# CederGroupHub/sparse-lm

Measured on NVIDIA B200. Metric: cv_grid_fits_per_sec, higher is better.
Workload: dtype f64

## Files before the change

include/sparselm_b200.h:

```cpp
#ifndef SPARSELM_B200_H
#define SPARSELM_B200_H

#include <stddef.h>
#include <stdint.h>

#ifdef __cplusplus
extern "C" {
#endif

#define SLM_MAX_FOLDS 16

typedef struct slm_ctx slm_ctx;

int slm_version(void);
int slm_create(int device, slm_ctx** out);
void slm_destroy(slm_ctx* ctx);
int slm_set_option(slm_ctx* ctx, const char* name, int value);
const char* slm_last_error(const slm_ctx* ctx);
int slm_sm_count(const slm_ctx* ctx);
int64_t slm_launch_count(const slm_ctx* ctx);
int64_t slm_tma_launch_count(const slm_ctx* ctx);
int slm_timing_enable(slm_ctx* ctx, int on);
int slm_timing_read(slm_ctx* ctx, int which, double* total_ms, int64_t* launches, double* flops);
int slm_timing_reset(slm_ctx* ctx);
// ... 104 lines not shown
                      const int32_t* K, const double* const* intercept_dev, int32_t rows_scaled,
                      double* const* yhat_dev, const int64_t* ldy, double* const* out_dev, void* stream);

int slm_cv_score_rows(slm_ctx* ctx, const double* Xa_dev, int64_t lda, int64_t p, int32_t n,
                      const int32_t* const* rows_dev, const int64_t* n_rows, const double* const* B_dev,
                      const int64_t* ldb, const int32_t* K, const double* const* intercept_dev, int32_t rows_scaled,
                      double* const* yhat_dev, const int64_t* ldy, double* const* out_dev, void* stream);

int slm_intercepts(slm_ctx* ctx, const double* G_dev, int64_t pa, int64_t p,
                   const double* B_dev, int64_t ldz, int32_t K, double* intercept_dev,
                   void* stream);

size_t slm_newton_workspace(int64_t p, int32_t n_groups, int32_t k, int n_folds);
int slm_newton_step(slm_ctx* ctx, const double* G_dev, int64_t g_stride, int64_t pa, int64_t p, int n_folds,
                    int32_t k, const int32_t* fold_host, const double* nobs_dev, double* X_dev,
                    const double* W2_dev, const double* D2_dev, const int32_t* gptr_dev, const int32_t* gid_dev,
                    int32_t n_groups, void* work_dev, size_t work_bytes, double* out_dev, void* stream);

int slm_newton_step_l1(slm_ctx* ctx, const double* G_dev, int64_t g_stride, int64_t pa, int64_t p, int n_folds,
                       int32_t k, const int32_t* fold_host, const double* nobs_dev, double* X_dev,
                       const double* W2_dev, const double* D2_dev, const double* W1_dev, const int32_t* gptr_dev,
                       const int32_t* gid_dev, int32_t n_groups, void* work_dev, size_t work_bytes, double* out_dev,
                       void* stream);

size_t slm_gram_cg_workspace(int64_t p);
int slm_gram_cg(slm_ctx* ctx, const double* G_dev, int64_t pa, int64_t p, const double* shift_dev,
                double tol, int32_t max_iter, void* work_dev, size_t work_bytes, double* X8_dev,
                int32_t* iters_host, double* relres_host, void* stream);

int slm_gram_apply(slm_ctx* ctx, const double* G_dev, int64_t g_stride, int64_t pa, int64_t p,
                   int n_folds, const int32_t* K, const double* Z_dev, int64_t ldz,
                   double* GZ_dev, void* stream);

size_t slm_rowsparse_workspace(int64_t p, int64_t ldz, int n_folds);
int slm_gram_apply_rowsparse(slm_ctx* ctx, const double* G_dev, int64_t g_stride, int64_t pa,
                             int64_t p, int n_folds, const int32_t* K, const double* Z_dev,
                             int64_t ldz, double* GZ_dev, int chunk_w, void* work_dev,
                             size_t work_bytes, void* stream);

int slm_apply_stats(slm_ctx* ctx, double* executed_flops, double* dense_flops);

int slm_group_whiten_factors(slm_ctx* ctx, const double* G_dev, int64_t pa, int64_t p,
                             const int32_t* gptr_dev, const int64_t* wptr_dev, int32_t n_groups,
                             const double* shift_dev, double* W_dev, double* scratch_dev,
                             int32_t* info_dev, void* stream);
int slm_gram_whiten(slm_ctx* ctx, const double* G_dev, int64_t pa, int64_t p,
                    const int32_t* gptr_dev, const int64_t* wptr_dev, int32_t n_groups,
                    const double* W_dev, const double* ridge_dev, double ridge_scale,
                    double* tmp_dev, double* Gout_dev, void* stream);
int slm_coef_unwhiten(slm_ctx* ctx, const double* Bg_dev, int64_t p, int64_t ldz, int32_t K,
                      const int32_t* gptr_dev, const int64_t* wptr_dev, int32_t n_groups,
                      const double* W_dev, double* B_dev, void* stream);

#ifdef __cplusplus
}
#endif
#endif
```

sparselm_b200/_build.py:

```python

from __future__ import annotations

import os
import shutil
import subprocess

_PKG = os.path.dirname(os.path.abspath(__file__))
CSRC = os.path.join(_PKG, "csrc")
LIB_DIR = os.path.join(_PKG, "lib")
LIB_PATH = os.path.join(LIB_DIR, "libsparselm_b200.so")
SOURCES = ["engine.cu"]
HEADERS = ["gemm_f64.cuh", "gemm_f64_tma.cuh", "solver_kernels.cuh", "whiten_kernels.cuh", "cg_kernels.cuh", "coop_kernels.cuh", "newton_kernels.cuh", os.path.join("..", "..", "include", "sparselm_b200.h")]

NVCC_FLAGS = [
    "-gencode", "arch=compute_100a,code=sm_100a",
    "-O3", "-lineinfo", "-std=c++17",
    "-Xcompiler", "-fPIC", "-shared",
]


def find_nvcc() -> str:
    nvcc = shutil.which("nvcc") or "/usr/local/cuda/bin/nvcc"
    if not os.path.exists(nvcc):
        raise RuntimeError("nvcc not found: the sparselm_b200 CUDA engine cannot be built")
    return nvcc


def is_stale() -> bool:
    if not os.path.exists(LIB_PATH):
        return True
    t = os.path.getmtime(LIB_PATH)
    deps = [os.path.join(CSRC, s) for s in SOURCES] + [os.path.join(CSRC, h) for h in HEADERS]
    return any(os.path.getmtime(d) > t for d in deps)


def build(force: bool = False, verbose: bool = False) -> str:
    if not force and not is_stale():
        return LIB_PATH
    os.makedirs(LIB_DIR, exist_ok=True)
    cmd = [find_nvcc(), *NVCC_FLAGS, "-o", LIB_PATH] + [os.path.join(CSRC, s) for s in SOURCES]
    if verbose:
        cmd.insert(1, "-Xptxas")
        cmd.insert(2, "-v")
    res = subprocess.run(cmd, capture_output=True, text=True)
    if res.returncode != 0:
# ... 9 lines not shown
```

sparselm_b200/_lib.py:

```python

from __future__ import annotations

import ctypes
import os

from . import _build

SLM_MAX_FOLDS = 16

c_i32, c_i64, c_dbl, c_vp, c_sz = (
    ctypes.c_int32, ctypes.c_int64, ctypes.c_double, ctypes.c_void_p, ctypes.c_size_t,
)


class SlmBatch(ctypes.Structure):

    _fields_ = [
        ("n_folds", c_i32),
        ("n_groups", c_i32),
        ("p", c_i64),
        ("pa", c_i64),
        ("ldz", c_i64),
        ("G_dev", c_vp),
        ("g_stride", c_i64),
# ... 35 lines not shown
    "slm_tma_launch_count": (c_i64, [c_vp]),
    "slm_timing_enable": (ctypes.c_int, [c_vp, ctypes.c_int]),
    "slm_timing_read": (ctypes.c_int, [c_vp, ctypes.c_int, ctypes.POINTER(c_dbl), ctypes.POINTER(c_i64), ctypes.POINTER(c_dbl)]),
    "slm_timing_reset": (ctypes.c_int, [c_vp]),
    "slm_padded_cols": (c_i64, [c_i64]),
    "slm_pack_design": (ctypes.c_int, [c_vp, c_vp, c_i64, c_vp, c_vp, c_vp, c_vp, c_i64, c_i64, c_vp, c_i64, c_vp]),
    "slm_gram_blocks": (ctypes.c_int, [c_vp, c_vp, c_i64, ctypes.POINTER(c_i64), ctypes.c_int, c_vp, c_vp]),
    "slm_gram_block_add": (ctypes.c_int, [c_vp, c_vp, c_i64, c_i64, c_i64, c_vp, c_vp]),
    "slm_gram_rows_update": (ctypes.c_int, [c_vp, c_vp, c_i64, c_i64, ctypes.c_int, ctypes.POINTER(c_i64), c_vp, c_vp, c_i64,
                                            ctypes.c_int, ctypes.c_int, c_vp]),
    "slm_gram_complement": (ctypes.c_int, [c_vp, c_vp, ctypes.c_int, c_i64, c_vp, c_vp]),
    "slm_tri_size": (c_i64, [c_i64]),
    "slm_tri_pack": (ctypes.c_int, [c_vp, c_vp, c_i64, c_i64, ctypes.c_int, c_vp, c_vp]),
    "slm_tri_unpack": (ctypes.c_int, [c_vp, c_vp, c_i64, ctypes.c_int, c_vp, c_i64, c_vp]),
    "slm_tri_complement": (ctypes.c_int, [c_vp, c_vp, c_i64, ctypes.c_int, c_vp, c_i64, c_vp]),
    "slm_gram_allreduce": (ctypes.c_int, [c_vp, c_vp, c_vp, c_i64, c_i64, ctypes.c_int, c_vp, c_vp]),
    "slm_allreduce_sum": (ctypes.c_int, [c_vp, c_vp, c_vp, c_i64, c_vp]),
    "slm_gather_results": (ctypes.c_int, [c_vp, c_vp, c_vp, c_vp, c_i64, c_vp]),
    "slm_tma_probe": (ctypes.c_int, [c_vp, c_vp, c_i64, c_i64, c_i32, c_i32, ctypes.POINTER(c_i32), c_vp, c_vp]),
    "slm_gram_center": (ctypes.c_int, [c_vp, c_vp, c_i64, c_i64, c_vp]),
    "slm_gram_gather": (ctypes.c_int, [c_vp, c_vp, c_i64, c_i64, c_vp, c_i64, c_vp, c_i64, c_vp]),
    "slm_lipschitz_workspace": (c_sz, [c_i64, ctypes.c_int]),
    "slm_lipschitz": (ctypes.c_int, [c_vp, c_vp, c_i64, c_i64, c_i64, ctypes.c_int, ctypes.c_int, c_vp, ctypes.POINTER(c_dbl), c_vp]),
    "slm_lipschitz_dev": (ctypes.c_int, [c_vp, c_vp, c_i64, c_i64, c_i64, ctypes.c_int, ctypes.c_int, c_vp, c_vp, c_vp]),
    "slm_solve_workspace": (c_sz, [c_i64, c_i64, ctypes.c_int, ctypes.c_int]),
    "slm_solve_batch": (ctypes.c_int, [c_vp, ctypes.POINTER(SlmBatch), c_vp]),
    "slm_adaptive_update": (ctypes.c_int, [c_vp, c_vp, c_i64, c_i64, c_i32, c_i32, c_vp, c_vp, c_vp, c_vp, c_vp, c_dbl, c_vp, c_vp, c_vp, c_vp]),
    "slm_fold_back": (ctypes.c_int, [c_vp, c_vp, c_vp, c_vp, c_i64, c_i64, c_i32, c_vp, c_vp]),
    "slm_cv_score": (ctypes.c_int, [c_vp, c_vp, c_i64, c_i64, c_i64, c_i64, c_vp, c_i64, c_i32, c_vp, c_i32, c_vp, c_vp, c_vp]),
    "slm_cv_score_many": (ctypes.c_int, [c_vp, c_vp, c_i64, c_i64, c_i32, c_vp, c_vp, c_vp, c_vp, c_vp, c_vp, c_i32, c_vp, c_vp, c_vp, c_vp]),
    "slm_cv_score_rows": (ctypes.c_int, [c_vp, c_vp, c_i64, c_i64, c_i32, c_vp, c_vp, c_vp, c_vp, c_vp, c_vp, c_i32, c_vp, c_vp, c_vp, c_vp]),
    "slm_intercepts": (ctypes.c_int, [c_vp, c_vp, c_i64, c_i64, c_vp, c_i64, c_i32, c_vp, c_vp]),
    "slm_gram_apply": (ctypes.c_int, [c_vp, c_vp, c_i64, c_i64, c_i64, ctypes.c_int, ctypes.POINTER(c_i32), c_vp, c_i64, c_vp, c_vp]),
    "slm_newton_workspace": (c_sz, [c_i64, c_i32, c_i32, ctypes.c_int]),
    "slm_newton_step": (ctypes.c_int, [c_vp, c_vp, c_i64, c_i64, c_i64, ctypes.c_int, c_i32, ctypes.POINTER(c_i32), c_vp, c_vp,
                                       c_vp, c_vp, c_vp, c_vp, c_i32, c_vp, c_sz, c_vp, c_vp]),
    "slm_newton_step_l1": (ctypes.c_int, [c_vp, c_vp, c_i64, c_i64, c_i64, ctypes.c_int, c_i32, ctypes.POINTER(c_i32), c_vp,
                                          c_vp, c_vp, c_vp, c_vp, c_vp, c_vp, c_i32, c_vp, c_sz, c_vp, c_vp]),
    "slm_gram_cg_workspace": (c_sz, [c_i64]),
    "slm_gram_cg": (ctypes.c_int, [c_vp, c_vp, c_i64, c_i64, c_vp, c_dbl, c_i32, c_vp, c_sz, c_vp, ctypes.POINTER(c_i32), ctypes.POINTER(c_dbl), c_vp]),
    "slm_rowsparse_workspace": (c_sz, [c_i64, c_i64, ctypes.c_int]),
    "slm_gram_apply_rowsparse": (ctypes.c_int, [c_vp, c_vp, c_i64, c_i64, c_i64, ctypes.c_int, ctypes.POINTER(c_i32), c_vp, c_i64, c_vp, ctypes.c_int, c_vp, c_sz, c_vp]),
    "slm_apply_stats": (ctypes.c_int, [c_vp, ctypes.POINTER(c_dbl), ctypes.POINTER(c_dbl)]),
    "slm_group_whiten_factors": (ctypes.c_int, [c_vp, c_vp, c_i64, c_i64, c_vp, c_vp, c_i32, c_vp, c_vp, c_vp, c_vp, c_vp]),
    "slm_gram_whiten": (ctypes.c_int, [c_vp, c_vp, c_i64, c_i64, c_vp, c_vp, c_i32, c_vp, c_vp, c_dbl, c_vp, c_vp, c_vp]),
    "slm_coef_unwhiten": (ctypes.c_int, [c_vp, c_vp, c_i64, c_i64, c_i32, c_vp, c_vp, c_i32, c_vp, c_vp, c_vp]),
}

_lib = None


def lib_path() -> str:
    return os.environ.get("SLM_B200_LIB") or _build.LIB_PATH


def load():
    global _lib
    if _lib is not None:
        return _lib
    path = lib_path()
    if not os.path.exists(path):
        raise RuntimeError(
            f"sparselm_b200 CUDA engine not built ({path} missing): run "
            "`python -c 'import __graft_entry__ as g; g.build()'` -- there is no CPU fallback"
        )
    lib = ctypes.CDLL(path)
# ... 7 lines not shown
```

sparselm_b200/csrc/engine.cu:

```cuda
#include <cuda_runtime.h>
#include <math.h>
#include <stdint.h>
#include <stdio.h>
#include <stdlib.h>
#include <string.h>

#include <algorithm>
#include <string>
#include <vector>

#include "../../include/sparselm_b200.h"
#include "gemm_f64.cuh"
#include "gemm_f64_tma.cuh"
#include "solver_kernels.cuh"
#include "whiten_kernels.cuh"
#include "cg_kernels.cuh"
#include "coop_kernels.cuh"
#include "newton_kernels.cuh"

using namespace slm;

enum { FAM_GRAM = 0, FAM_APPLY = 1, FAM_PROX = 2, FAM_GAP = 3, FAM_SCORE = 4, FAM_LIPS = 5, FAM_COUNT = 6 };

struct Family {
    std::vector<cudaEvent_t> ev;
    std::vector<cudaEvent_t> pool;
    double ms = 0.0;
    double flops = 0.0;
    int64_t n = 0;
};

constexpr int kMaxScount = 4096;
constexpr int kMaxDevices = 64;

struct slm_ctx {
    int device = 0;
    int sm_count = 148;
    std::string err;
    int64_t launches = 0;
    int64_t tma_launches = 0;
    bool timing = false;
    bool newton_smem_set = false;
    Family fam[FAM_COUNT];
    int* d_counter = nullptr;
    int* h_counter = nullptr;
    int* d_flags = nullptr;
    int n_flags_cap = 0;
    unsigned long long* d_stat = nullptr;
    unsigned long long* h_stat = nullptr;
    unsigned long long* d_ratio = nullptr;
    unsigned long long* h_ratio = nullptr;
    int* h_scount = nullptr;
    double* h_scal = nullptr;
    double apply_exec_flops = 0.0;
    double apply_dense_flops = 0.0;
    int chunk_w = 32;
    bool dense_apply = false;
    bool small_fused = true;
    bool coop = true;
    bool trace = false;
    int coop_max_smem = 0;
    int max_cluster = 16;
    int force_sparse_shape = -1;
    int force_apply_shape = -1;
    int force_syrk_shape = -1;
    bool fused_prox = true;
    bool prox2 = false;
    int tma_mask = 7 + 8;
    void* encode = nullptr;
};

static int fail(slm_ctx* ctx, int code, const std::string& msg) {
    if (ctx) ctx->err = msg;
    return code;
}
#define CUDA_OK(call)                                                                      \
    do {                                                                                   \
        cudaError_t e__ = (call);                                                          \
        if (e__ != cudaSuccess)                                                            \
            return fail(ctx, 100 + (int)e__,                                               \
                        std::string(#call) + ": " + cudaGetErrorString(e__));              \
    } while (0)
#define LAUNCH_OK(name)                                                                    \
    do {                                                                                   \
        cudaError_t e__ = cudaGetLastError();                                              \
        if (e__ != cudaSuccess)                                                            \
            return fail(ctx, 100 + (int)e__, std::string(name) + ": " + cudaGetErrorString(e__)); \
        ctx->launches++;                                                                   \
    } while (0)

struct FamTimer {
    slm_ctx* ctx;
    int fam;
    cudaStream_t s;
    cudaEvent_t e0 = nullptr, e1 = nullptr;
    FamTimer(slm_ctx* c, int f, cudaStream_t st, double flops) : ctx(c), fam(f), s(st) {
        Family& F = ctx->fam[fam];
        F.flops += flops;
        F.n += 1;
// ... 328 lines not shown
        memset(&b, 0, sizeof(b));
        ProblemDims pd[kMaxGemmProblems];
        double flops = 0.0;
        b.n_problems = nf;
        if (g_stride % pa == 0) {
            b.baseP = G;
            b.rowsP = (int64_t)(F - 1) * (g_stride / pa) + pa;
            b.baseQ = Z;
            b.rowsQ = (int64_t)F * p;
        }
        for (int i = 0; i < nf; ++i) {
            int f = f0 + i;
            GemmProblem& pr = b.pr[i];
            pr.P = G + (int64_t)f * g_stride;
            pr.Q = Z + (int64_t)f * p * ldz;
            pr.C = GZ + (int64_t)f * p * ldz;
            pr.ldp = pa;
            pr.ldq = ldz;
            pr.ldc = ldz;
            pr.M = (int)p;
            pr.N = (int)std::min<int64_t>(round_up(K[f], 8), ldz);
            pr.Kd = (int)p;
            pd[i] = {pr.M, pr.N};
            flops += 2.0 * (double)p * (double)p * (double)K[f];
        }
        int sid = pick_shape(kApplyShapes, kNumApplyShapes, pd, nf, ctx->sm_count);
        if (ctx->force_apply_shape >= 0 && ctx->force_apply_shape < kNumApplyShapes) sid = ctx->force_apply_shape;
        FamTimer tm(ctx, family, s, algo_flops >= 0 ? algo_flops : flops);
        cudaError_t e = launch_apply_shape(ctx, sid, b, s);
        if (e != cudaSuccess) return fail(ctx, 100 + (int)e, std::string("gram apply: ") + cudaGetErrorString(e));
        ctx->launches++;
    }
    return 0;
}

static int apply_rowsparse(slm_ctx* ctx, const SolveDev& sp, const int32_t* K, const double* Z, double* GZ,
                           int chunk_w, int ncc, int* sidx, int* scount, cudaStream_t s, double algo_flops) {
    const int F = sp.F;
    const int64_t p = sp.p, ldz = sp.ldz;
    support_list_kernel<<<dim3((unsigned)ncc, (unsigned)F), 1024, 0, s>>>(sp, chunk_w / SC, ncc, sidx, scount,
                                                                          ctx->d_stat);
    LAUNCH_OK("support_list_kernel");
    GemmBatch b;
    ProblemDims pd[kMaxGemmProblems];
    int np = 0;
    double dense = 0.0;
    bool first = true;
    auto flush = [&]() -> int {
        if (np == 0) return 0;
        b.n_problems = np;
        if (sp.g_stride % sp.pa == 0) {
            b.baseP = sp.G;
            b.rowsP = (int64_t)(F - 1) * (sp.g_stride / sp.pa) + sp.pa;
            b.baseQ = Z;
            b.rowsQ = (int64_t)F * p;
        }
        int sid = pick_shape(kSparseShapes, kNumSparseShapes, pd, np, ctx->sm_count);
        if (ctx->force_sparse_shape >= 0 && ctx->force_sparse_shape < 14) sid = ctx->force_sparse_shape;
        FamTimer tm(ctx, FAM_APPLY, s, first ? std::max(algo_flops, 0.0) : 0.0);
        first = false;
        cudaError_t e = launch_sparse_shape(ctx, sid, b, s);
        if (e != cudaSuccess) return fail(ctx, 100 + (int)e, std::string("row-sparse apply: ") + cudaGetErrorString(e));
        ctx->launches++;
        np = 0;
        return 0;
    };
// ... 151 lines not shown
        if (gl < s) red[gl][c] += red[gl + s][c];
        __syncthreads();
    }
    T r = red[0][c];
    __syncthreads();
    return r;
}

__global__ void init_cols_kernel(double* theta, double* tmom, int* flag, int* colmap, int* status, int* n_iter,
                                 const int* skip, long long n, int ldz) {
    long long i = (long long)blockIdx.x * blockDim.x + threadIdx.x;
    if (i >= n) return;
    theta[i] = theta[n + i] = 0.0;
    tmom[i] = tmom[n + i] = 1.0;
    colmap[i] = (int)(i % ldz);
    if (skip && skip[i]) {
        flag[i] = 3;
        return;
    }
    flag[i] = 0;
    if (status) status[i] = -1;
    if (n_iter) n_iter[i] = 0;
}

constexpr int PN_LANES = 128;
__global__ void __launch_bounds__(8 * PN_LANES) power_norm_kernel(double* __restrict__ V, const double* __restrict__ W,
                                                                  int p, double* __restrict__ lam, int init) {
    const int f = blockIdx.x;
    const int c = threadIdx.x & 7, r = threadIdx.x >> 3;
    double* Vf = V + (long long)f * p * 8;
    const double* Wf = W + (long long)f * p * 8;
    __shared__ double red[3][PN_LANES][8];
    if (init) {
        for (int j = r; j < p; j += PN_LANES) {
            unsigned h = (unsigned)(j * 8 + c) * 2654435761u + 12345u * (unsigned)(f + 1);
            h ^= h >> 15;
            h *= 2246822519u;
            h ^= h >> 13;
            Vf[(long long)j * 8 + c] = ((double)(h & 0xffffff) / 8388608.0) - 1.0;
        }
        if (threadIdx.x == 0) lam[f] = 0.0;
        return;
    }
    double vw = 0.0, ww = 0.0, vv = 0.0;
    for (int j = r; j < p; j += PN_LANES) {
        double v = Vf[(long long)j * 8 + c], w = Wf[(long long)j * 8 + c];
        vw += v * w;
        ww += w * w;
        vv += v * v;
    }
    red[0][r][c] = vw;
    red[1][r][c] = ww;
    red[2][r][c] = vv;
    __syncthreads();
    for (int s = PN_LANES / 2; s > 0; s >>= 1) {
        if (r < s) {
            red[0][r][c] += red[0][r + s][c];
            red[1][r][c] += red[1][r + s][c];
            red[2][r][c] += red[2][r + s][c];
        }
        __syncthreads();
    }
    vw = red[0][0][c];
    ww = red[1][0][c];
    vv = red[2][0][c];
    if (threadIdx.x == 0) {
        double best = lam[f];
        for (int cc = 0; cc < 8; ++cc) {
            double q = red[2][0][cc] > 0.0 ? red[0][0][cc] / red[2][0][cc] : 0.0;
            best = fmax(best, q);
        }
        lam[f] = best;
    }
// ... 131 lines not shown
extern "C" {

int slm_version(void) { return 1; }

int64_t slm_padded_cols(int64_t p) { return round_up(p + 2, 8); }

int slm_create(int device, slm_ctx** out) {
    if (!out) return 1;
    *out = nullptr;
    int ndev = 0;
    cudaError_t e = cudaGetDeviceCount(&ndev);
    if (e != cudaSuccess || ndev == 0) return 2;
    if (device < 0 || device >= ndev) return 3;
    if (cudaSetDevice(device) != cudaSuccess) return 4;
    slm_ctx* ctx = new slm_ctx();
    ctx->device = device;
    cudaDeviceProp prop;
    if (cudaGetDeviceProperties(&prop, device) != cudaSuccess) {
        delete ctx;
        return 5;
    }
    ctx->sm_count = prop.multiProcessorCount;
    if (const char* e = getenv("SLM_FORCE_APPLY_SHAPE")) ctx->force_apply_shape = atoi(e);
    if (const char* e = getenv("SLM_FORCE_SYRK_SHAPE")) ctx->force_syrk_shape = atoi(e);
    if (const char* e = getenv("SLM_FORCE_SPARSE_SHAPE")) ctx->force_sparse_shape = atoi(e);
    if (const char* e = getenv("SLM_CHUNK_W")) ctx->chunk_w = std::max(8, atoi(e) / 8 * 8);
    if (const char* e = getenv("SLM_DENSE_APPLY")) ctx->dense_apply = atoi(e) != 0;
    if (const char* e = getenv("SLM_SMALL_FUSED")) ctx->small_fused = atoi(e) != 0;
    if (const char* e = getenv("SLM_COOP")) ctx->coop = atoi(e) != 0;
    if (const char* e = getenv("SLM_TRACE")) ctx->trace = atoi(e) != 0;
    if (const char* e = getenv("SLM_TMA")) ctx->tma_mask = atoi(e);
    if (const char* e = getenv("SLM_PROX2")) ctx->prox2 = atoi(e) != 0;
    if (const char* e = getenv("SLM_FUSED_PROX")) ctx->fused_prox = atoi(e) != 0;
    {
        void* fn = nullptr;
        cudaDriverEntryPointQueryResult qres;
        if (cudaGetDriverEntryPoint("cuTensorMapEncodeTiled", &fn, cudaEnableDefault, &qres) == cudaSuccess &&
            qres == cudaDriverEntryPointSuccess)
            ctx->encode = fn;
        else
            cudaGetLastError();
    }
    ctx->coop_max_smem = (int)prop.sharedMemPerBlockOptin;
    if (!prop.cooperativeLaunch) ctx->coop = false;
    if (const char* e = getenv("SLM_MAX_CLUSTER")) ctx->max_cluster = std::max(1, std::min(16, atoi(e)));
    if (ctx->max_cluster > 8) {
        if (cudaFuncSetAttribute(fista_coop_kernel<true, true>, cudaFuncAttributeNonPortableClusterSizeAllowed, 1) !=
                cudaSuccess ||
            cudaFuncSetAttribute(fista_coop_kernel<false, true>, cudaFuncAttributeNonPortableClusterSizeAllowed, 1) !=
                cudaSuccess) {
            cudaGetLastError();
            ctx->max_cluster = 8;
        }
    }
    ctx->n_flags_cap = 1 << 20;
    if (cudaMalloc(&ctx->d_flags, sizeof(int) * (size_t)ctx->n_flags_cap) != cudaSuccess ||
        cudaMalloc(&ctx->d_counter, sizeof(int) * SLM_MAX_FOLDS) != cudaSuccess ||
        cudaMalloc(&ctx->d_stat, sizeof(unsigned long long)) != cudaSuccess ||
        cudaMallocHost(&ctx->h_stat, sizeof(unsigned long long)) != cudaSuccess ||
        cudaMalloc(&ctx->d_ratio, sizeof(unsigned long long)) != cudaSuccess ||
        cudaMallocHost(&ctx->h_ratio, sizeof(unsigned long long)) != cudaSuccess ||
        cudaMallocHost(&ctx->h_scount, sizeof(int) * kMaxScount) != cudaSuccess ||
        cudaMallocHost(&ctx->h_scal, sizeof(double) * 8) != cudaSuccess ||
        cudaMallocHost(&ctx->h_counter, sizeof(int) * SLM_MAX_FOLDS) != cudaSuccess) {
        delete ctx;
        return 6;
// ... 8 lines not shown
    for (auto& F : ctx->fam) {
        for (auto e : F.ev) cudaEventDestroy(e);
        for (auto e : F.pool) cudaEventDestroy(e);
    }
    if (ctx->d_counter) cudaFree(ctx->d_counter);
    if (ctx->d_stat) cudaFree(ctx->d_stat);
    if (ctx->h_stat) cudaFreeHost(ctx->h_stat);
    if (ctx->d_ratio) cudaFree(ctx->d_ratio);
    if (ctx->h_ratio) cudaFreeHost(ctx->h_ratio);
    if (ctx->h_scount) cudaFreeHost(ctx->h_scount);
    if (ctx->h_scal) cudaFreeHost(ctx->h_scal);
    if (ctx->d_flags) cudaFree(ctx->d_flags);
    if (ctx->h_counter) cudaFreeHost(ctx->h_counter);
    delete ctx;
}

int slm_set_option(slm_ctx* ctx, const char* name, int value) {
    if (!ctx || !name) return 1;
    const std::string nm(name);
    if (nm == "coop")
        ctx->coop = value != 0;
    else if (nm == "small_fused")
        ctx->small_fused = value != 0;
    else if (nm == "dense_apply")
        ctx->dense_apply = value != 0;
    else if (nm == "chunk_w")
        ctx->chunk_w = std::max(8, value / 8 * 8);
    else if (nm == "tma")
        ctx->tma_mask = value;
    else if (nm == "prox2")
        ctx->prox2 = value != 0;
    else if (nm == "fused_prox")
        ctx->fused_prox = value != 0;
    else if (nm == "force_apply_shape")
        ctx->force_apply_shape = value;
    else if (nm == "force_sparse_shape")
        ctx->force_sparse_shape = value;
    else if (nm == "force_syrk_shape")
        ctx->force_syrk_shape = value;
    else
        return fail(ctx, 1, "slm_set_option: unknown option " + nm);
    return 0;
}

const char* slm_last_error(const slm_ctx* ctx) { return ctx ? ctx->err.c_str() : "null context"; }
int slm_sm_count(const slm_ctx* ctx) { return ctx ? ctx->sm_count : 0; }
int64_t slm_launch_count(const slm_ctx* ctx) { return ctx ? ctx->launches : 0; }
int64_t slm_tma_launch_count(const slm_ctx* ctx) { return ctx ? ctx->tma_launches : 0; }

int slm_timing_enable(slm_ctx* ctx, int on) {
    if (!ctx) return 1;
    ctx->timing = on != 0;
    return 0;
}
static void timing_collect(slm_ctx* ctx) {
    for (auto& F : ctx->fam) {
        for (size_t i = 0; i + 1 < F.ev.size(); i += 2) {
            float ms = 0.f;
            cudaEventSynchronize(F.ev[i + 1]);
            if (cudaEventElapsedTime(&ms, F.ev[i], F.ev[i + 1]) == cudaSuccess) F.ms += ms;
            F.pool.push_back(F.ev[i]);
            F.pool.push_back(F.ev[i + 1]);
        }
        F.ev.clear();
    }
}
// ... 183 lines not shown
    if (n_blocks < 1 || n_blocks > SLM_MAX_FOLDS) return fail(ctx, 1, "slm_tri_complement: n_blocks out of range");
    if (pa <= 0) return 0;
    dim3 grid((unsigned)((pa + 255) / 256), (unsigned)pa);
    tri_complement_kernel<<<grid, 256, 0, (cudaStream_t)stream>>>(buf, slm_tri_size(pa), pa, n_blocks, G, g_stride);
    LAUNCH_OK("tri_complement_kernel");
    return 0;
}

int slm_gram_center(slm_ctx* ctx, double* G, int64_t pa, int64_t p, void* stream) {
    if (!ctx || !G) return fail(ctx, 1, "slm_gram_center: null argument");
    dim3 grid((unsigned)((p + 1 + 255) / 256), (unsigned)(p + 1));
    gram_center_kernel<<<grid, 256, 0, (cudaStream_t)stream>>>(G, pa, (int)p);
    LAUNCH_OK("gram_center_kernel");
    return 0;
}

int slm_gram_gather(slm_ctx* ctx, const double* G, int64_t pa, int64_t p, const int32_t* idx, int64_t pe,
                    double* Ge, int64_t pae, void* stream) {
    if (!ctx || !G || !idx || !Ge) return fail(ctx, 1, "slm_gram_gather: null argument");
    if (pae < pe + 2) return fail(ctx, 1, "slm_gram_gather: pae too small");
    dim3 grid((unsigned)((pae + 255) / 256), (unsigned)pae);
    gram_gather_kernel<<<grid, 256, 0, (cudaStream_t)stream>>>(G, pa, (int)p, idx, (int)pe, Ge, pae);
    LAUNCH_OK("gram_gather_kernel");
    return 0;
}

int slm_gram_apply(slm_ctx* ctx, const double* G, int64_t g_stride, int64_t pa, int64_t p, int n_folds,
                   const int32_t* K, const double* Z, int64_t ldz, double* GZ, void* stream) {
    if (!ctx || !G || !K || !Z || !GZ) return fail(ctx, 1, "slm_gram_apply: null argument");
    if (ldz % 8 || pa % 2) return fail(ctx, 1, "slm_gram_apply: ldz must be a multiple of 8, pa even");
    return apply_batched(ctx, G, g_stride, pa, p, n_folds, K, Z, ldz, GZ, (cudaStream_t)stream);
}

size_t slm_gram_cg_workspace(int64_t p) { return (size_t)(3 * 8 * p + p + 8) * sizeof(double); }

int slm_gram_cg(slm_ctx* ctx, const double* G, int64_t pa, int64_t p, const double* shift, double tol,
                int32_t max_iter, void* work, size_t work_bytes, double* X8, int32_t* iters_host,
                double* relres_host, void* stream) {
    if (!ctx || !G || !work || !X8) return fail(ctx, 1, "slm_gram_cg: null argument");
    if (pa % 2 || pa < p + 1) return fail(ctx, 1, "slm_gram_cg: pa must be even and hold the X^T y row");
    if (work_bytes < slm_gram_cg_workspace(p)) return fail(ctx, 1, "slm_gram_cg: workspace too small");
    if (!(tol > 0.0)) return fail(ctx, 1, "slm_gram_cg: tol must be positive");
    cudaStream_t s = (cudaStream_t)stream;
    double* D8 = (double*)work;
    double* GD8 = D8 + 8 * p;
    double* GX8 = GD8 + 8 * p;
    double* R = GX8 + 8 * p;
    double* sc = R + p;
    const int32_t K1 = 1;
    CUDA_OK(cudaMemsetAsync(work, 0, slm_gram_cg_workspace(p), s));
    CUDA_OK(cudaMemsetAsync(X8, 0, sizeof(double) * 8 * (size_t)p, s));
    cg_start_kernel<<<1, CG_T, 0, s>>>(G, pa, (int)p, X8, nullptr, shift, R, D8, sc);
    LAUNCH_OK("cg_start_kernel");
    auto scalars = [&]() -> int {
        CUDA_OK(cudaMemcpyAsync(ctx->h_scal, sc, sizeof(double) * 3, cudaMemcpyDeviceToHost, s));
        CUDA_OK(cudaStreamSynchronize(s));
        return 0;
    };
    int it = 0, restarts = 0;
    double rel = 0.0;
    const int check = 8;
    while (true) {
        bool conv = false;
        for (; it < max_iter; ++it) {
            if (it % check == 0) {
                if (int rc = scalars()) return rc;
                const double rs = ctx->h_scal[0], cc = ctx->h_scal[1];
                if (!(rs == rs)) return fail(ctx, 7, "slm_gram_cg: non-finite residual");
                rel = cc > 0.0 ? sqrt(rs / cc) : 0.0;
                if (rel <= tol) {
                    conv = true;
                    break;
                }
            }
            int rc = apply_batched(ctx, G, pa * pa, pa, p, 1, &K1, D8, 8, GD8, s, -1.0, FAM_LIPS);
            if (rc) return rc;
            cg_step_kernel<<<1, CG_T, 0, s>>>((int)p, X8, R, D8, GD8, shift, sc);
            LAUNCH_OK("cg_step_kernel");
        }
        int rc = apply_batched(ctx, G, pa * pa, pa, p, 1, &K1, X8, 8, GX8, s, -1.0, FAM_LIPS);
        if (rc) return rc;
        cg_start_kernel<<<1, CG_T, 0, s>>>(G, pa, (int)p, X8, GX8, shift, R, D8, sc);
        LAUNCH_OK("cg_start_kernel");
        if (int rc2 = scalars()) return rc2;
        rel = ctx->h_scal[1] > 0.0 ? sqrt(ctx->h_scal[0] / ctx->h_scal[1]) : 0.0;
        if (rel <= 4.0 * tol || it >= max_iter || (conv && ++restarts > 3)) break;
    }
    if (iters_host) *iters_host = it;
    if (relres_host) *relres_host = rel;
    return 0;
}

size_t slm_rowsparse_workspace(int64_t p, int64_t ldz, int n_folds) {
    size_t nblk = (size_t)ldz / 8;
    return (size_t)n_folds * nblk * ((size_t)p + 1) * sizeof(int) + (size_t)n_folds * (size_t)p * nblk + 64;
}

int slm_gram_apply_rowsparse(slm_ctx* ctx, const double* G, int64_t g_stride, int64_t pa, int64_t p, int n_folds,
                             const int32_t* K, const double* Z, int64_t ldz, double* GZ, int chunk_w, void* work,
                             size_t work_bytes, void* stream) {
    if (!ctx || !G || !K || !Z || !GZ || !work) return fail(ctx, 1, "slm_gram_apply_rowsparse: null argument");
    if (ldz % 8 || pa % 2) return fail(ctx, 1, "slm_gram_apply_rowsparse: ldz must be a multiple of 8, pa even");
    if (n_folds < 1 || n_folds > SLM_MAX_FOLDS) return fail(ctx, 1, "slm_gram_apply_rowsparse: n_folds out of range");
    if (chunk_w < 8 || chunk_w % 8) return fail(ctx, 1, "slm_gram_apply_rowsparse: chunk_w must be a multiple of 8");
    if (work_bytes < slm_rowsparse_workspace(p, ldz, n_folds))
        return fail(ctx, 1, "slm_gram_apply_rowsparse: workspace too small");
    cudaStream_t s = (cudaStream_t)stream;
    const int ncc = (int)((ldz + chunk_w - 1) / chunk_w);
    SolveDev sp;
    memset(&sp, 0, sizeof(sp));
    sp.F = n_folds;
    sp.p = (int)p;
    sp.ldz = ldz;
    sp.pa = pa;
    sp.g_stride = g_stride;
    sp.G = G;
    sp.nblk = (int)(ldz / SC);
    int* sidx = (int*)work;
    int* scount = sidx + (size_t)n_folds * ncc * p;
    sp.zflag = (unsigned char*)(sidx + (size_t)n_folds * sp.nblk * (p + 1));
    for (int f = 0; f < n_folds; ++f) {
        if (K[f] < 0 || K[f] > ldz) return fail(ctx, 1, "slm_gram_apply_rowsparse: K[f] out of range");
        sp.K[f] = K[f];
    }
    const dim3 zgrid((unsigned)(((long long)p * sp.nblk + 255) / 256), (unsigned)n_folds);
    zflags_kernel<<<zgrid, 256, 0, s>>>(sp, Z);
    LAUNCH_OK("zflags_kernel");
    return apply_rowsparse(ctx, sp, K, Z, GZ, chunk_w, ncc, sidx, scount, s, -1.0);
}

size_t slm_lipschitz_workspace(int64_t p, int n_grams) {
    return (size_t)(2 * (int64_t)n_grams * p * 8 + n_grams) * sizeof(double);
}

static int lipschitz_run(slm_ctx* ctx, const double* G, int64_t g_stride, int64_t pa, int64_t p, int n_grams,
                         int iters, void* work, double** lam_out, cudaStream_t s) {
    double* V = (double*)work;
    double* W = V + (int64_t)n_grams * p * 8;
    double* lam = W + (int64_t)n_grams * p * 8;
    std::vector<int32_t> K(n_grams, 8);
    power_norm_kernel<<<n_grams, 8 * PN_LANES, 0, s>>>(V, W, (int)p, lam, 1);
    LAUNCH_OK("power_norm_kernel(init)");
    for (int it = 0; it < iters; ++it) {
        int rc = apply_batched(ctx, G, g_stride, pa, p, n_grams, K.data(), V, 8, W, s, -1.0, FAM_LIPS);
        if (rc) return rc;
        power_norm_kernel<<<n_grams, 8 * PN_LANES, 0, s>>>(V, W, (int)p, lam, 0);
        LAUNCH_OK("power_norm_kernel");
    }
    *lam_out = lam;
    return 0;
}

int slm_lipschitz(slm_ctx* ctx, const double* G, int64_t g_stride, int64_t pa, int64_t p, int n_grams,
                  int iters, void* work, double* lam_host, void* stream) {
    if (!ctx || !G || !work || !lam_host) return fail(ctx, 1, "slm_lipschitz: null argument");
    cudaStream_t s = (cudaStream_t)stream;
    double* lam = nullptr;
    int rc = lipschitz_run(ctx, G, g_stride, pa, p, n_grams, iters, work, &lam, s);
    if (rc) return rc;
    CUDA_OK(cudaMemcpyAsync(lam_host, lam, sizeof(double) * n_grams, cudaMemcpyDeviceToHost, s));
    CUDA_OK(cudaStreamSynchronize(s));
    return 0;
}

int slm_lipschitz_dev(slm_ctx* ctx, const double* G, int64_t g_stride, int64_t pa, int64_t p, int n_grams,
                      int iters, void* work, double* lam_dev, void* stream) {
    if (!ctx || !G || !work || !lam_dev) return fail(ctx, 1, "slm_lipschitz_dev: null argument");
    cudaStream_t s = (cudaStream_t)stream;
    double* lam = nullptr;
    int rc = lipschitz_run(ctx, G, g_stride, pa, p, n_grams, iters, work, &lam, s);
    if (rc) return rc;
    CUDA_OK(cudaMemcpyAsync(lam_dev, lam, sizeof(double) * n_grams, cudaMemcpyDeviceToDevice, s));
    return 0;
}

static void chunk_geometry(const slm_ctx* ctx, int64_t ldz, int* w, int* ncc) {
    int cw = ctx ? ctx->chunk_w : 32;
    cw = std::max(8, cw / 8 * 8);
    *w = cw;
    *ncc = (int)((ldz + cw - 1) / cw);
}

// ... 962 lines not shown
```

sparselm_b200/engine.py:

```python

from __future__ import annotations

import ctypes
import os
import sys
from dataclasses import dataclass, field

import numpy as np

from . import _lib

__all__ = ["Engine", "PenaltyGrid", "FoldData", "SplitData", "EngineError", "get_engine", "plan_splits", "split_chunks"]


class EngineError(RuntimeError):
    pass


def _round_up(x, m):
    return (x + m - 1) // m * m


@dataclass
class PenaltyGrid:
# ... 361 lines not shown
            lam = (ctypes.c_double * nf)()
            self._ck(self.lib.slm_lipschitz(self.h, self._ptr(Gs[f0]), pa * pa, pa, p, nf, iters,
                                            self._ptr(work), lam, self.stream), "slm_lipschitz")
            out[f0:f0 + nf] = np.frombuffer(lam, dtype=np.float64, count=nf)
        return out

    def lipschitz_device(self, G, p, iters=None):
        torch = self.torch
        pa = G.shape[-1]
        Gs = G.reshape(-1, pa, pa)
        F = Gs.shape[0]
        out = torch.empty(F, dtype=torch.float64, device=self.device)
        iters = self.LIPSCHITZ_ITERS if iters is None else iters
        for f0 in range(0, F, _lib.SLM_MAX_FOLDS):
            nf = min(F - f0, _lib.SLM_MAX_FOLDS)
            nbytes = self.lib.slm_lipschitz_workspace(p, nf)
            work = torch.empty(nbytes, dtype=torch.uint8, device=self.device)
            self._ck(self.lib.slm_lipschitz_dev(self.h, self._ptr(Gs[f0]), pa * pa, pa, p, nf, iters,
                                                self._ptr(work), ctypes.c_void_p(out.data_ptr() + 8 * f0),
                                                self.stream), "slm_lipschitz_dev")
        return out

    def gram_apply(self, G, p, K, Z):
        torch = self.torch
        pa = G.shape[-1]
        Gs = G.reshape(-1, pa, pa)
        F = Gs.shape[0]
        ldz = Z.shape[-1]
        GZ = torch.zeros_like(Z)
        Karr = (ctypes.c_int32 * F)(*[int(k) for k in K])
        self._ck(self.lib.slm_gram_apply(self.h, self._ptr(Gs), pa * pa, pa, p, F, Karr, self._ptr(Z), ldz,
                                         self._ptr(GZ), self.stream), "slm_gram_apply")
        return GZ

    def gram_cg(self, G, p, tol=1e-13, max_iter=None, shift=None):
        torch = self.torch
        pa = G.shape[-1]
        if max_iter is None:
            max_iter = 10 * int(p) + 100
        nbytes = self.lib.slm_gram_cg_workspace(p)
        work = torch.empty(nbytes, dtype=torch.uint8, device=self.device)
        X8 = torch.empty((p, 8), dtype=torch.float64, device=self.device)
        iters, rel = ctypes.c_int32(0), ctypes.c_double(0.0)
        self._ck(self.lib.slm_gram_cg(self.h, self._ptr(G), pa, p, self._ptr(shift), float(tol), int(max_iter),
                                      self._ptr(work), nbytes,
                                      self._ptr(X8), ctypes.byref(iters), ctypes.byref(rel), self.stream),
                 "slm_gram_cg")
        return X8, int(iters.value), float(rel.value)

    def gram_apply_rowsparse(self, G, p, K, Z, chunk_w=32):
        torch = self.torch
        pa = G.shape[-1]
        Gs = G.reshape(-1, pa, pa)
        F = Gs.shape[0]
        ldz = Z.shape[-1]
        GZ = torch.zeros_like(Z)
        Karr = (ctypes.c_int32 * F)(*[int(k) for k in K])
        nbytes = self.lib.slm_rowsparse_workspace(p, ldz, F)
        work = torch.empty(nbytes, dtype=torch.uint8, device=self.device)
        self._ck(self.lib.slm_gram_apply_rowsparse(self.h, self._ptr(Gs), pa * pa, pa, p, F, Karr, self._ptr(Z), ldz,
                                                   self._ptr(GZ), int(chunk_w), self._ptr(work), nbytes,
                                                   self.stream), "slm_gram_apply_rowsparse")
        return GZ

    def apply_stats(self):
        ex, de = ctypes.c_double(), ctypes.c_double()
# ... 745 lines not shown
```

Before: 18360.

## Add symmetric Gram apply kernel fusing power-iteration norms for Lipschitz and CG

New measurement: 17760 (median of 6 runs). 3.3% lower.

```diff
diff --git a/include/sparselm_b200.h b/include/sparselm_b200.h
--- a/include/sparselm_b200.h
+++ b/include/sparselm_b200.h
@@ -160,6 +160,9 @@
                    int n_folds, const int32_t* K, const double* Z_dev, int64_t ldz,
                    double* GZ_dev, void* stream);
 
+int slm_gram_apply_sym8(slm_ctx* ctx, const double* G_dev, int64_t g_stride, int64_t pa, int64_t p,
+                        int n_grams, const double* V_dev, double* W_dev, void* stream);
+
 size_t slm_rowsparse_workspace(int64_t p, int64_t ldz, int n_folds);
 int slm_gram_apply_rowsparse(slm_ctx* ctx, const double* G_dev, int64_t g_stride, int64_t pa,
                              int64_t p, int n_folds, const int32_t* K, const double* Z_dev,
diff --git a/sparselm_b200/_build.py b/sparselm_b200/_build.py
--- a/sparselm_b200/_build.py
+++ b/sparselm_b200/_build.py
@@ -10,7 +10,7 @@
 LIB_DIR = os.path.join(_PKG, "lib")
 LIB_PATH = os.path.join(LIB_DIR, "libsparselm_b200.so")
 SOURCES = ["engine.cu"]
-HEADERS = ["gemm_f64.cuh", "gemm_f64_tma.cuh", "solver_kernels.cuh", "whiten_kernels.cuh", "cg_kernels.cuh", "coop_kernels.cuh", "newton_kernels.cuh", os.path.join("..", "..", "include", "sparselm_b200.h")]
+HEADERS = ["gemm_f64.cuh", "gemm_f64_tma.cuh", "solver_kernels.cuh", "whiten_kernels.cuh", "cg_kernels.cuh", "coop_kernels.cuh", "newton_kernels.cuh", "sym_apply.cuh", os.path.join("..", "..", "include", "sparselm_b200.h")]
 
 NVCC_FLAGS = [
     "-gencode", "arch=compute_100a,code=sm_100a",
diff --git a/sparselm_b200/_lib.py b/sparselm_b200/_lib.py
--- a/sparselm_b200/_lib.py
+++ b/sparselm_b200/_lib.py
@@ -91,6 +91,7 @@
     "slm_cv_score_rows": (ctypes.c_int, [c_vp, c_vp, c_i64, c_i64, c_i32, c_vp, c_vp, c_vp, c_vp, c_vp, c_vp, c_i32, c_vp, c_vp, c_vp, c_vp]),
     "slm_intercepts": (ctypes.c_int, [c_vp, c_vp, c_i64, c_i64, c_vp, c_i64, c_i32, c_vp, c_vp]),
     "slm_gram_apply": (ctypes.c_int, [c_vp, c_vp, c_i64, c_i64, c_i64, ctypes.c_int, ctypes.POINTER(c_i32), c_vp, c_i64, c_vp, c_vp]),
+    "slm_gram_apply_sym8": (ctypes.c_int, [c_vp, c_vp, c_i64, c_i64, c_i64, ctypes.c_int, c_vp, c_vp, c_vp]),
     "slm_newton_workspace": (c_sz, [c_i64, c_i32, c_i32, ctypes.c_int]),
     "slm_newton_step": (ctypes.c_int, [c_vp, c_vp, c_i64, c_i64, c_i64, ctypes.c_int, c_i32, ctypes.POINTER(c_i32), c_vp, c_vp,
                                        c_vp, c_vp, c_vp, c_vp, c_i32, c_vp, c_sz, c_vp, c_vp]),
diff --git a/sparselm_b200/csrc/engine.cu b/sparselm_b200/csrc/engine.cu
--- a/sparselm_b200/csrc/engine.cu
+++ b/sparselm_b200/csrc/engine.cu
@@ -17,6 +17,7 @@
 #include "cg_kernels.cuh"
 #include "coop_kernels.cuh"
 #include "newton_kernels.cuh"
+#include "sym_apply.cuh"
 
 using namespace slm;
 
@@ -65,6 +66,7 @@
     int force_apply_shape = -1;
     int force_syrk_shape = -1;
     bool fused_prox = true;
+    bool sym_apply = true;
     bool prox2 = false;
     int tma_mask = 7 + 8;
     void* encode = nullptr;
@@ -459,6 +461,43 @@
         ctx->launches++;
     }
     return 0;
+}
+
+static int sym_strip(const slm_ctx* ctx, int64_t p, int n_grams) {
+    return (int64_t)n_grams * ((p + 63) / 64) >= ctx->sm_count ? 64 : 32;
+}
+static bool sym_ok(const double* G, int64_t g_stride, int64_t pa) {
+    return G && ((uintptr_t)G & 15) == 0 && pa % 2 == 0 && g_stride % 2 == 0;
+}
+static int sym_apply_launch(slm_ctx* ctx, const SymApplyArgs& a, int n_grams, int bs, cudaStream_t s) {
+    FamTimer tm(ctx, FAM_LIPS, s, 2.0 * (double)a.p * (double)a.p * 8.0 * n_grams);
+    const dim3 grid((unsigned)a.nb, (unsigned)n_grams);
+    if (bs == 64)
+        sym_apply8_kernel<64><<<grid, kSymThreads, 0, s>>>(a);
+    else
+        sym_apply8_kernel<32><<<grid, kSymThreads, 0, s>>>(a);
+    LAUNCH_OK("sym_apply8_kernel");
+    return 0;
+}
+static int sym_apply_plain(slm_ctx* ctx, const double* G, int64_t g_stride, int64_t pa, int64_t p, int n_grams,
+                           const double* V, double* W, cudaStream_t s) {
+    const int bs = sym_strip(ctx, p, n_grams);
+    SymApplyArgs a;
+    memset(&a, 0, sizeof(a));
+    a.G = G;
+    a.g_stride = g_stride;
+    a.pa = pa;
+    a.p = (int)p;
+    a.nb = (int)((p + bs - 1) / bs);
+    a.V = V;
+    a.W = W;
+    a.mode = SYM_PLAIN;
+    return sym_apply_launch(ctx, a, n_grams, bs, s);
+}
+static int apply8(slm_ctx* ctx, const double* G, int64_t pa, int64_t p, const double* Z, double* GZ, cudaStream_t s) {
+    if (ctx->sym_apply && sym_ok(G, pa * pa, pa)) return sym_apply_plain(ctx, G, pa * pa, pa, p, 1, Z, GZ, s);
+    const int32_t K1 = 1;
+    return apply_batched(ctx, G, pa * pa, pa, p, 1, &K1, Z, 8, GZ, s, -1.0, FAM_LIPS);
 }
 
 static int apply_rowsparse(slm_ctx* ctx, const SolveDev& sp, const int32_t* K, const double* Z, double* GZ,
@@ -676,13 +715,7 @@
     const double* Wf = W + (long long)f * p * 8;
     __shared__ double red[3][PN_LANES][8];
     if (init) {
-        for (int j = r; j < p; j += PN_LANES) {
-            unsigned h = (unsigned)(j * 8 + c) * 2654435761u + 12345u * (unsigned)(f + 1);
-            h ^= h >> 15;
-            h *= 2246822519u;
-            h ^= h >> 13;
-            Vf[(long long)j * 8 + c] = ((double)(h & 0xffffff) / 8388608.0) - 1.0;
-        }
+        for (int j = r; j < p; j += PN_LANES) Vf[(long long)j * 8 + c] = power_init_value(j, c, f);
         if (threadIdx.x == 0) lam[f] = 0.0;
         return;
     }
@@ -880,6 +913,7 @@
     if (const char* e = getenv("SLM_TMA")) ctx->tma_mask = atoi(e);
     if (const char* e = getenv("SLM_PROX2")) ctx->prox2 = atoi(e) != 0;
     if (const char* e = getenv("SLM_FUSED_PROX")) ctx->fused_prox = atoi(e) != 0;
+    if (const char* e = getenv("SLM_SYM_APPLY")) ctx->sym_apply = atoi(e) != 0;
     {
         void* fn = nullptr;
         cudaDriverEntryPointQueryResult qres;
@@ -954,6 +988,8 @@
         ctx->prox2 = value != 0;
     else if (nm == "fused_prox")
         ctx->fused_prox = value != 0;
+    else if (nm == "sym_apply")
+        ctx->sym_apply = value != 0;
     else if (nm == "force_apply_shape")
         ctx->force_apply_shape = value;
     else if (nm == "force_sparse_shape")
@@ -1203,6 +1239,15 @@
     return apply_batched(ctx, G, g_stride, pa, p, n_folds, K, Z, ldz, GZ, (cudaStream_t)stream);
 }
 
+int slm_gram_apply_sym8(slm_ctx* ctx, const double* G, int64_t g_stride, int64_t pa, int64_t p, int n_grams,
+                        const double* V, double* W, void* stream) {
+    if (!ctx || !G || !V || !W) return fail(ctx, 1, "slm_gram_apply_sym8: null argument");
+    if (!sym_ok(G, g_stride, pa) || ((uintptr_t)V & 15))
+        return fail(ctx, 1, "slm_gram_apply_sym8: G and V must be 16-byte aligned, pa and g_stride even");
+    if (p < 1 || pa < p || n_grams < 1 || n_grams > 65535) return fail(ctx, 1, "slm_gram_apply_sym8: bad sizes");
+    return sym_apply_plain(ctx, G, g_stride, pa, p, n_grams, V, W, (cudaStream_t)stream);
+}
+
 size_t slm_gram_cg_workspace(int64_t p) { return (size_t)(3 * 8 * p + p + 8) * sizeof(double); }
 
 int slm_gram_cg(slm_ctx* ctx, const double* G, int64_t pa, int64_t p, const double* shift, double tol,
@@ -1218,7 +1263,6 @@
     double* GX8 = GD8 + 8 * p;
     double* R = GX8 + 8 * p;
     double* sc = R + p;
-    const int32_t K1 = 1;
     CUDA_OK(cudaMemsetAsync(work, 0, slm_gram_cg_workspace(p), s));
     CUDA_OK(cudaMemsetAsync(X8, 0, sizeof(double) * 8 * (size_t)p, s));
     cg_start_kernel<<<1, CG_T, 0, s>>>(G, pa, (int)p, X8, nullptr, shift, R, D8, sc);
@@ -1244,12 +1288,12 @@
                     break;
                 }
             }
-            int rc = apply_batched(ctx, G, pa * pa, pa, p, 1, &K1, D8, 8, GD8, s, -1.0, FAM_LIPS);
+            int rc = apply8(ctx, G, pa, p, D8, GD8, s);
             if (rc) return rc;
             cg_step_kernel<<<1, CG_T, 0, s>>>((int)p, X8, R, D8, GD8, shift, sc);
             LAUNCH_OK("cg_step_kernel");
         }
-        int rc = apply_batched(ctx, G, pa * pa, pa, p, 1, &K1, X8, 8, GX8, s, -1.0, FAM_LIPS);
+        int rc = apply8(ctx, G, pa, p, X8, GX8, s);
         if (rc) return rc;
         cg_start_kernel<<<1, CG_T, 0, s>>>(G, pa, (int)p, X8, GX8, shift, R, D8, sc);
         LAUNCH_OK("cg_start_kernel");
@@ -1301,7 +1345,8 @@
 }
 
 size_t slm_lipschitz_workspace(int64_t p, int n_grams) {
-    return (size_t)(2 * (int64_t)n_grams * p * 8 + n_grams) * sizeof(double);
+    const int64_t strips = (p + 31) / 32;
+    return (size_t)(2 * (int64_t)n_grams * p * 8 + n_grams + 2 * (int64_t)n_grams * kSymNQ * strips) * sizeof(double);
 }
 
 static int lipschitz_run(slm_ctx* ctx, const double* G, int64_t g_stride, int64_t pa, int64_t p, int n_grams,
@@ -1309,6 +1354,36 @@
     double* V = (double*)work;
     double* W = V + (int64_t)n_grams * p * 8;
     double* lam = W + (int64_t)n_grams * p * 8;
+    *lam_out = lam;
+    if (n_grams <= 0 || p <= 0) return 0;
+    if (ctx->sym_apply && sym_ok(G, g_stride, pa)) {
+        const int bs = sym_strip(ctx, p, n_grams);
+        double* part0 = lam + n_grams;
+        double* part1 = part0 + (int64_t)n_grams * kSymNQ * ((p + 31) / 32);
+        if (iters <= 0) {
+            CUDA_OK(cudaMemsetAsync(lam, 0, sizeof(double) * n_grams, s));
+            return 0;
+        }
+        SymApplyArgs a;
+        memset(&a, 0, sizeof(a));
+        a.G = G;
+        a.g_stride = g_stride;
+        a.pa = pa;
+        a.p = (int)p;
+        a.nb = (int)((p + bs - 1) / bs);
+        a.lam = lam;
+        for (int it = 0; it < iters; ++it) {
+            a.mode = it == 0 ? SYM_POWER_FIRST : SYM_POWER;
+            a.V = it == 0 ? nullptr : (it & 1 ? V : W);
+            a.W = it & 1 ? W : V;
+            a.part_in = it & 1 ? part0 : part1;
+            a.part_out = it & 1 ? part1 : part0;
+            if (int rc = sym_apply_launch(ctx, a, n_grams, bs, s)) return rc;
+        }
+        sym_power_final_kernel<<<n_grams, kSymThreads, 0, s>>>(a.part_out, a.nb, lam);
+        LAUNCH_OK("sym_power_final_kernel");
+        return 0;
+    }
     std::vector<int32_t> K(n_grams, 8);
     power_norm_kernel<<<n_grams, 8 * PN_LANES, 0, s>>>(V, W, (int)p, lam, 1);
     LAUNCH_OK("power_norm_kernel(init)");
@@ -1318,7 +1393,6 @@
         power_norm_kernel<<<n_grams, 8 * PN_LANES, 0, s>>>(V, W, (int)p, lam, 0);
         LAUNCH_OK("power_norm_kernel");
     }
-    *lam_out = lam;
     return 0;
 }
 
diff --git a/sparselm_b200/csrc/sym_apply.cuh b/sparselm_b200/csrc/sym_apply.cuh
--- /dev/null
+++ b/sparselm_b200/csrc/sym_apply.cuh
@@ -0,0 +1,224 @@
+#pragma once
+#include <cuda_runtime.h>
+#include <stdint.h>
+
+#include "gemm_f64.cuh"
+
+namespace slm {
+
+constexpr int kSymThreads = 128;
+constexpr int kSymBK = 16;
+constexpr int kSymStages = 4;
+constexpr int kSymVLD = 12;
+constexpr int kSymNQ = 24;
+
+enum { SYM_PLAIN = 0, SYM_POWER_FIRST = 1, SYM_POWER = 2 };
+
+struct SymApplyArgs {
+    const double* G;
+    long long g_stride, pa;
+    int p;
+    int nb;
+    const double* V;
+    double* W;
+    const double* part_in;
+    double* part_out;
+    double* lam;
+    int mode;
+};
+
+__device__ __forceinline__ double power_init_value(int j, int c, int f) {
+    unsigned h = (unsigned)(j * 8 + c) * 2654435761u + 12345u * (unsigned)(f + 1);
+    h ^= h >> 15;
+    h *= 2246822519u;
+    h ^= h >> 13;
+    return ((double)(h & 0xffffff) / 8388608.0) - 1.0;
+}
+
+__device__ __forceinline__ void cp_async16n(void* smem_dst, const void* gsrc, int bytes) {
+    unsigned dst = (unsigned)__cvta_generic_to_shared(smem_dst);
+    asm volatile("cp.async.cg.shared.global [%0], [%1], 16, %2;\n" ::"r"(dst), "l"(gsrc), "r"(bytes));
+}
+__device__ __forceinline__ void cp_async8(void* smem_dst, const void* gsrc, bool valid) {
+    unsigned dst = (unsigned)__cvta_generic_to_shared(smem_dst);
+    asm volatile("cp.async.ca.shared.global [%0], [%1], 8, %2;\n" ::"r"(dst), "l"(gsrc), "r"(valid ? 8 : 0));
+}
+
+__device__ __forceinline__ void sym_reduce_partials(const double* __restrict__ pin, int nb, double* out) {
+    const int lane = threadIdx.x & 31, warp = threadIdx.x >> 5;
+    for (int q = warp; q < kSymNQ; q += kSymThreads / 32) {
+        double s = 0.0;
+        for (int t = lane; t < nb; t += 32) s += pin[(long long)q * nb + t];
+        for (int o = 16; o > 0; o >>= 1) s += __shfl_xor_sync(0xffffffffu, s, o);
+        if (lane == 0) out[q] = s;
+    }
+    __syncthreads();
+}
+__device__ __forceinline__ void sym_update_lam(const double* red, double* lam) {
+    double best = *lam;
+    for (int c = 0; c < 8; ++c) {
+        const double q = red[16 + c] > 0.0 ? red[c] / red[16 + c] : 0.0;
+        best = fmax(best, q);
+    }
+    *lam = best;
+}
+
+template <int BS>
+__global__ void __launch_bounds__(kSymThreads) sym_apply8_kernel(const SymApplyArgs a) {
+    constexpr int SL = BS / kSymBK;
+    constexpr int LDR = kSymBK + 4;
+    constexpr int LDC = BS + 4;
+    constexpr int A_SZ = BS * LDR > kSymBK * LDC ? BS * LDR : kSymBK * LDC;
+    constexpr int ST_SZ = A_SZ + kSymBK * kSymVLD;
+    constexpr int MT = BS / 8;
+    static_assert(BS % kSymBK == 0 && 4 * BS * 8 <= kSymStages * ST_SZ, "strip / stage geometry");
+    __shared__ __align__(16) double sm[kSymStages * ST_SZ];
+    __shared__ double s_red[kSymNQ];
+    __shared__ double s_part[kSymThreads / 32][kSymNQ];
+
+    const int tid = threadIdx.x, lane = tid & 31, warp = tid >> 5;
+    const int lk = lane & 3, lx = lane >> 2;
+    const int i = blockIdx.x, f = blockIdx.y, nb = a.nb, p = a.p, mode = a.mode;
+    const long long pa = a.pa;
+    const double* __restrict__ G = a.G + (long long)f * a.g_stride;
+    const double* __restrict__ V = a.V ? a.V + (long long)f * p * 8 : nullptr;
+    const int i0 = i * BS;
+
+    if (mode == SYM_POWER) {
+        sym_reduce_partials(a.part_in + (long long)f * kSymNQ * nb, nb, s_red);
+        if (i == 0 && tid == 0) sym_update_lam(s_red, a.lam + f);
+    } else if (mode == SYM_POWER_FIRST && i == 0 && tid == 0) {
+        a.lam[f] = 0.0;
+    }
+    auto col_scale = [&](int c) {
+        if (mode != SYM_POWER) return 1.0;
+        const double ww = s_red[8 + c];
+        return ww > 0.0 ? rsqrt(ww) : 0.0;
+    };
+    const double sc = col_scale(lx);
+
+    auto load_slab = [&](int s) {
+        const int t = s / SL, q = s % SL;
+        const int j = (t + nb - i) % nb;
+        const int k0 = j * BS + q * kSymBK;
+        double* A = sm + (s % kSymStages) * ST_SZ;
+        if (j > i) {
+#pragma unroll
+            for (int id = tid; id < BS * kSymBK / 2; id += kSymThreads) {
+                const int m = id / (kSymBK / 2), kk = (id % (kSymBK / 2)) * 2;
+                const int r = i0 + m, c = k0 + kk;
+                const int bytes = r < p ? (c + 1 < p ? 16 : (c < p ? 8 : 0)) : 0;
+                cp_async16n(A + m * LDR + kk, bytes ? G + (long long)r * pa + c : G, bytes);
+            }
+        } else if (j < i) {
+#pragma unroll
+            for (int id = tid; id < kSymBK * BS / 2; id += kSymThreads) {
+                const int kk = id / (BS / 2), m = (id % (BS / 2)) * 2;
+                const int r = k0 + kk, c = i0 + m;
+                const int bytes = r < p ? (c + 1 < p ? 16 : (c < p ? 8 : 0)) : 0;
+                cp_async16n(A + kk * LDC + m, bytes ? G + (long long)r * pa + c : G, bytes);
+            }
+        } else {
+#pragma unroll
+            for (int id = tid; id < BS * kSymBK; id += kSymThreads) {
+                const int m = id / kSymBK, kk = id % kSymBK;
+                const int r = i0 + m, c = k0 + kk;
+                const bool ok = r < p && c < p;
+                const double* src = r <= c ? G + (long long)r * pa + c : G + (long long)c * pa + r;
+                cp_async8(A + m * LDR + kk, ok ? src : G, ok);
+            }
+        }
+        if (mode != SYM_POWER_FIRST && tid < kSymBK * 4) {
+            const int kk = tid >> 2, c = (tid & 3) * 2, r = k0 + kk;
+            cp_async16n(A + A_SZ + kk * kSymVLD + c, r < p ? V + (long long)r * 8 + c : V, r < p ? 16 : 0);
+        }
+    };
+
+    double acc[MT][2];
+#pragma unroll
+    for (int mt = 0; mt < MT; ++mt) acc[mt][0] = acc[mt][1] = 0.0;
+
+    const int n_slabs = nb * SL;
+#pragma unroll
+    for (int s = 0; s < kSymStages - 1; ++s) {
+        if (s < n_slabs) load_slab(s);
+        cp_async_commit();
+    }
+    for (int s = 0; s < n_slabs; ++s) {
+        cp_async_wait<kSymStages - 2>();
+        __syncthreads();
+        if (s + kSymStages - 1 < n_slabs) load_slab(s + kSymStages - 1);
+        cp_async_commit();
+        const double* A = sm + (s % kSymStages) * ST_SZ;
+        const int t = s / SL, q = s % SL;
+        const int j = (t + nb - i) % nb;
+        const int kk = warp * 4 + lk;
+        double b;
+        if (mode == SYM_POWER_FIRST) {
+            const int kg = j * BS + q * kSymBK + kk;
+            b = kg < p ? power_init_value(kg, lx, f) : 0.0;
+        } else {
+            b = A[A_SZ + kk * kSymVLD + lx] * sc;
+        }
+        if (j < i) {
+#pragma unroll
+            for (int mt = 0; mt < MT; ++mt) dmma_m8n8k4(acc[mt][0], acc[mt][1], A[kk * LDC + mt * 8 + lx], b);
+        } else {
+#pragma unroll
+            for (int mt = 0; mt < MT; ++mt) dmma_m8n8k4(acc[mt][0], acc[mt][1], A[(mt * 8 + lx) * LDR + kk], b);
+        }
+    }
+    cp_async_wait<0>();
+    __syncthreads();
+
+    double* red = sm;
+#pragma unroll
+    for (int mt = 0; mt < MT; ++mt) {
+        const int m = mt * 8 + lx;
+        red[(warp * BS + m) * 8 + 2 * lk] = acc[mt][0];
+        red[(warp * BS + m) * 8 + 2 * lk + 1] = acc[mt][1];
+    }
+    __syncthreads();
+    const int c = tid & 7;
+    const double scc = col_scale(c);
+    double* Wf = a.W + (long long)f * p * 8;
+    double vw = 0.0, ww = 0.0, vv = 0.0;
+#pragma unroll
+    for (int m = tid >> 3; m < BS; m += kSymThreads / 8) {
+        const double x = red[m * 8 + c] + red[(BS + m) * 8 + c] + red[(2 * BS + m) * 8 + c] + red[(3 * BS + m) * 8 + c];
+        const int r = i0 + m;
+        if (r < p) {
+            Wf[(long long)r * 8 + c] = x;
+            if (mode != SYM_PLAIN) {
+                const double v = mode == SYM_POWER_FIRST ? power_init_value(r, c, f) : V[(long long)r * 8 + c] * scc;
+                vw += v * x;
+                ww += x * x;
+                vv += v * v;
+            }
+        }
+    }
+    if (mode == SYM_PLAIN) return;
+    for (int o = 8; o < 32; o <<= 1) {
+        vw += __shfl_xor_sync(0xffffffffu, vw, o);
+        ww += __shfl_xor_sync(0xffffffffu, ww, o);
+        vv += __shfl_xor_sync(0xffffffffu, vv, o);
+    }
+    if (lane < 8) {
+        s_part[warp][lane] = vw;
+        s_part[warp][8 + lane] = ww;
+        s_part[warp][16 + lane] = vv;
+    }
+    __syncthreads();
+    if (tid < kSymNQ)
+        a.part_out[((long long)f * kSymNQ + tid) * nb + i] = s_part[0][tid] + s_part[1][tid] + s_part[2][tid] + s_part[3][tid];
+}
+
+__global__ void __launch_bounds__(kSymThreads) sym_power_final_kernel(const double* __restrict__ part, int nb,
+                                                                     double* __restrict__ lam) {
+    __shared__ double s_red[kSymNQ];
+    const int f = blockIdx.x;
+    sym_reduce_partials(part + (long long)f * kSymNQ * nb, nb, s_red);
+    if (threadIdx.x == 0) sym_update_lam(s_red, lam + f);
+}
+
+}
diff --git a/sparselm_b200/engine.py b/sparselm_b200/engine.py
--- a/sparselm_b200/engine.py
+++ b/sparselm_b200/engine.py
@@ -417,6 +417,15 @@
         self._ck(self.lib.slm_gram_apply(self.h, self._ptr(Gs), pa * pa, pa, p, F, Karr, self._ptr(Z), ldz,
                                          self._ptr(GZ), self.stream), "slm_gram_apply")
         return GZ
+
+    def gram_apply_sym8(self, G, p, V, pa=None, g_stride=None):
+        pa = G.shape[-1] if pa is None else pa
+        n = V.shape[0]
+        g_stride = pa * pa if g_stride is None else g_stride
+        W = self.torch.zeros_like(V)
+        self._ck(self.lib.slm_gram_apply_sym8(self.h, self._ptr(G), g_stride, pa, p, n, self._ptr(V),
+                                              self._ptr(W), self.stream), "slm_gram_apply_sym8")
+        return W
 
     def gram_cg(self, G, p, tol=1e-13, max_iter=None, shift=None):
         torch = self.torch
```
